# jialeli1/From-Voxel-to-Point

Measured on AMD Instinct MI355X. Metric: point clouds/sec fwd+bwd (FV2P, KITTI shape) at 1/2/4/8 MI355X, higher is better.
Workload: dtype f32

## Files before the change

from-voxel-to-point_amd/csrc/roi_pool.hip:

```cpp
#include "common.hpp"
#include "../../include/fv2p_math.h"

namespace fv2p {

FV2P_HD int pt_in_box3d(const float* pt, const float* box, float margin, float* local_x, float* local_y) {
  const float x = pt[0], y = pt[1], z = pt[2];
  const float cx = box[0], cy = box[1], cz = box[2];
  const float dx = box[3], dy = box[4], dz = box[5], rz = box[6];
  if (static_cast<double>(fabsf(z - cz)) > static_cast<double>(dz) / 2.0) return 0;
  const float sx = x - cx, sy = y - cy;
  const float cosa = fv2p_cosf(-rz), sina = fv2p_sinf(-rz);
  const float lx = sx * cosa + sy * (-sina);
  const float ly = sx * sina + sy * cosa;
  *local_x = lx;
  *local_y = ly;
  const bool in_x = static_cast<double>(fabsf(lx)) < static_cast<double>(dx) / 2.0 + static_cast<double>(margin);
  const bool in_y = static_cast<double>(fabsf(ly)) < static_cast<double>(dy) / 2.0 + static_cast<double>(margin);
  return in_x && in_y;
}

constexpr float kMarginGpu = 1e-5f;
constexpr float kMarginCpu = 1e-2f;

__global__ __launch_bounds__(256) void points_in_boxes_k(int boxes_num, int pts_num, const float* __restrict__ boxes,
// ... 9 lines not shown
  int idx = -1;
  float lx, ly;
  for (int k = 0; k < boxes_num; ++k)
    if (pt_in_box3d(pt, sbox + k * 7, kMarginGpu, &lx, &ly)) { idx = k; break; }
  out[static_cast<int64_t>(b) * pts_num + i] = idx;
}

constexpr int kRoiPoolWaves = 16;
__device__ __forceinline__ int roi_pool_select(int pts_num, int sampled, int row, const float* __restrict__ xyz_b, const float* box, int* sidx,
                                               int* wave_cnt, float* __restrict__ dst, int* __restrict__ empty_flag) {
  constexpr int T = kRoiPoolWaves * 64;
  const int lane = threadIdx.x & 63, w = threadIdx.x >> 6;
  int total = 0;
  for (int base = 0; base < pts_num && total < sampled; base += T) {
    const int i = base + threadIdx.x;
    int in = 0;
    if (i < pts_num) {
      const float* p = xyz_b + static_cast<int64_t>(i) * 3;
      const float pt[3] = {p[0], p[1], p[2]};
      float lx, ly;
      in = pt_in_box3d(pt, box, kMarginGpu, &lx, &ly);
    }
    const uint64_t vote = __ballot(in);
    if (lane == 0) wave_cnt[w] = __popcll(vote);
    __syncthreads();
    int pos = total + __popcll(vote & lanemask_lt()), all = 0;
#pragma unroll
    for (int ww = 0; ww < kRoiPoolWaves; ++ww) { const int c = wave_cnt[ww]; if (ww < w) pos += c; all += c; }
    if (in && pos < sampled) sidx[pos] = i;
    total += all;
    __syncthreads();
  }
  const int cnt = total < sampled ? total : sampled;
  if (threadIdx.x == 0) *empty_flag = (cnt == 0) ? 1 : 0;
  if (cnt == 0)
    for (int e = threadIdx.x; e < sampled * row; e += T) dst[e] = 0.f;
  return cnt;
}

__global__ __launch_bounds__(kRoiPoolWaves * 64) void roipoint_pool_k(int pts_num, int boxes_num, int feat_len, int sampled, const float* __restrict__ xyz,
                                                       const float* __restrict__ boxes3d, const float* __restrict__ feats,
                                                       float* __restrict__ pooled, int* __restrict__ empty_flag) {
  extern __shared__ int sidx[];
  __shared__ int wave_cnt[kRoiPoolWaves];
  const int m = blockIdx.x, b = blockIdx.y;
  const int lane = threadIdx.x & 63, w = threadIdx.x >> 6;
  float box[7];
  for (int j = 0; j < 7; ++j) box[j] = boxes3d[(static_cast<int64_t>(b) * boxes_num + m) * 7 + j];
  const int row = 3 + feat_len;
  float* dst = pooled + (static_cast<int64_t>(b) * boxes_num + m) * sampled * row;
  const int cnt = roi_pool_select(pts_num, sampled, row, xyz + static_cast<int64_t>(b) * pts_num * 3, box, sidx, wave_cnt, dst,
                                  empty_flag + static_cast<int64_t>(b) * boxes_num + m);
  if (cnt == 0) return;
  const float* fx = xyz + static_cast<int64_t>(b) * pts_num * 3;
  const float* ff = feats + static_cast<int64_t>(b) * pts_num * feat_len;
  for (int s0 = 4 * w; s0 < sampled; s0 += 4 * kRoiPoolWaves) {
    int src[4];
#pragma unroll
    for (int u = 0; u < 4; ++u) { const int sl = s0 + u < sampled ? s0 + u : sampled - 1; src[u] = sidx[sl < cnt ? sl : sl % cnt]; }
    for (int j0 = 0; j0 < row; j0 += 128) {
      float v[4][2];
#pragma unroll
      for (int u = 0; u < 4; ++u)
#pragma unroll
        for (int q = 0; q < 2; ++q) {
          const int j = j0 + 64 * q + lane;
          v[u][q] = j < 3 ? fx[static_cast<int64_t>(src[u]) * 3 + j] : (j < row ? ff[static_cast<int64_t>(src[u]) * feat_len + (j - 3)] : 0.f);
// ... 30 lines not shown
  const float ca = cosf(-roi[6]), sa = sinf(-roi[6]);
  const float* fs = score + static_cast<int64_t>(b) * pts_num;
  const float* ff = feats + static_cast<int64_t>(b) * pts_num * feat_len;
  for (int s0 = 4 * w; s0 < sampled; s0 += 4 * kRoiPoolWaves) {
    int src[4];
    float head[4];
#pragma unroll
    for (int u = 0; u < 4; ++u) { const int sl = s0 + u < sampled ? s0 + u : sampled - 1; src[u] = sidx[sl < cnt ? sl : sl % cnt]; }
#pragma unroll
    for (int u = 0; u < 4; ++u) {
      const float* p = fx + static_cast<int64_t>(src[u]) * 3;
      const float x = p[0], y = p[1], z = p[2], sc = fs[src[u]];
      const float dx = x - roi[0], dy = y - roi[1];
      head[u] = lane == 0 ? dx * ca - dy * sa : (lane == 1 ? dx * sa + dy * ca : (lane == 2 ? z - roi[2] : (lane == 3 ? sc : sqrtf(x * x + y * y + z * z) / depth_norm - 0.5f)));
    }
    for (int j0 = 0; j0 < row; j0 += 128) {
      float v[4][2];
#pragma unroll
      for (int u = 0; u < 4; ++u)
#pragma unroll
        for (int q = 0; q < 2; ++q) {
          const int j = j0 + 64 * q + lane;
          const float f = (j >= 5 && j < row) ? ff[static_cast<int64_t>(src[u]) * feat_len + (j - 5)] : 0.f;
          v[u][q] = j < 5 ? head[u] : f;
        }
#pragma unroll
      for (int u = 0; u < 4; ++u)
#pragma unroll
        for (int q = 0; q < 2; ++q) {
          const int j = j0 + 64 * q + lane;
          if (j < row && s0 + u < sampled) dst[static_cast<int64_t>(s0 + u) * row + j] = v[u][q];
        }
    }
  }
}

__global__ __launch_bounds__(64) void roiaware_collect_k(int pts_num, int max_pts, int out_x, int out_y, int out_z,
                                                         const float* __restrict__ rois, const float* __restrict__ pts,
                                                         int* __restrict__ pts_idx_of_voxels) {
  extern __shared__ int s_cnt[];
  const int box_idx = blockIdx.x, lane = threadIdx.x;
  const int nvox = out_x * out_y * out_z;
  for (int e = lane; e < nvox; e += 64) s_cnt[e] = 0;
  __builtin_amdgcn_wave_barrier();
  float box[7];
  for (int j = 0; j < 7; ++j) box[j] = rois[box_idx * 7 + j];
  int* vox = pts_idx_of_voxels + static_cast<int64_t>(box_idx) * nvox * max_pts;
  const int max_num = max_pts - 1;
  const float dx = box[3], dy = box[4], dz = box[5];
  const float x_res = dx / out_x, y_res = dy / out_y, z_res = dz / out_z;
  for (int base = 0; base < pts_num; base += 64) {
    const int i = base + lane;
    int in = 0, v = -1;
    if (i < pts_num) {
      const float pt[3] = {pts[i * 3], pts[i * 3 + 1], pts[i * 3 + 2]};
      float lx = 0.f, ly = 0.f;
      in = pt_in_box3d(pt, box, kMarginGpu, &lx, &ly);
      if (in) {
        const float lz = pt[2] - box[2];
        int xi = static_cast<int>((lx + dx / 2) / x_res);
        int yi = static_cast<int>((ly + dy / 2) / y_res);
        int zi = static_cast<int>((lz + dz / 2) / z_res);
        xi = min(max(xi, 0), out_x - 1);
        yi = min(max(yi, 0), out_y - 1);
        zi = min(max(zi, 0), out_z - 1);
        v = (xi * out_y + yi) * out_z + zi;
// ... 119 lines not shown
                                    fv2p_stream_t stream_) {
  hipStream_t stream = static_cast<hipStream_t>(stream_);
  FV2P_REQUIRE(batch >= 0 && pts_num >= 0 && boxes_num >= 0 && feature_len >= 0 && sampled_pts_num >= 1, FV2P_EINVAL,
               "roipoint_pool3d: bad sizes");
  if (batch == 0 || boxes_num == 0) return 0;
  FV2P_REQUIRE(boxes3d && pooled_features && pooled_empty_flag && (xyz || pts_num == 0) && (pts_feature || feature_len == 0 || pts_num == 0),
               FV2P_EINVAL, "roipoint_pool3d: null pointer");
  FV2P_REQUIRE(static_cast<size_t>(sampled_pts_num) * 4 <= 60000, FV2P_ELIMIT, "roipoint_pool3d: sampled_pts_num > 15000");
  hipLaunchKernelGGL(roipoint_pool_k, dim3(boxes_num, batch), dim3(kRoiPoolWaves * 64), sampled_pts_num * sizeof(int), stream, pts_num, boxes_num,
                     feature_len, sampled_pts_num, xyz, boxes3d, pts_feature, pooled_features, pooled_empty_flag);
  FV2P_LAUNCH_CHECK();
  return 0;
}

extern "C" int fv2p_roipoint_pool3d_frame(const float* xyz, const float* pts_score, const float* pts_feature, const float* boxes3d,
                                          const float* rois, int batch, int pts_num, int boxes_num, int feature_len, int sampled_pts_num,
                                          float depth_normalizer, float* pooled_features, int* pooled_empty_flag, fv2p_stream_t stream_) {
  hipStream_t stream = static_cast<hipStream_t>(stream_);
  FV2P_REQUIRE(batch >= 0 && pts_num >= 0 && boxes_num >= 0 && feature_len >= 0 && sampled_pts_num >= 1, FV2P_EINVAL,
               "roipoint_pool3d_frame: bad sizes");
  FV2P_REQUIRE(depth_normalizer > 0.f, FV2P_EINVAL, "roipoint_pool3d_frame: depth_normalizer must be positive");
  if (batch == 0 || boxes_num == 0) return 0;
  FV2P_REQUIRE(boxes3d && rois && pooled_features && pooled_empty_flag && ((xyz && pts_score) || pts_num == 0) &&
               (pts_feature || feature_len == 0 || pts_num == 0), FV2P_EINVAL, "roipoint_pool3d_frame: null pointer");
  FV2P_REQUIRE(static_cast<size_t>(sampled_pts_num) * 4 <= 60000, FV2P_ELIMIT, "roipoint_pool3d_frame: sampled_pts_num > 15000");
  FV2P_REQUIRE(static_cast<int64_t>(sampled_pts_num) * (5 + feature_len) < (1ll << 31), FV2P_ELIMIT, "roipoint_pool3d_frame: a RoI's rows exceed 2^31 values");
  hipLaunchKernelGGL(roipoint_pool_frame_k, dim3(boxes_num, batch), dim3(kRoiPoolWaves * 64), sampled_pts_num * sizeof(int), stream, pts_num,
                     boxes_num, feature_len, sampled_pts_num, depth_normalizer, xyz, pts_score, pts_feature, boxes3d, rois, pooled_features,
                     pooled_empty_flag);
  FV2P_LAUNCH_CHECK();
  return 0;
}

extern "C" int fv2p_roiaware_pool3d_fwd(const float* rois, const float* pts, const float* pts_feature, int boxes_num, int pts_num,
                                        int channels, int max_pts_each_voxel, int out_x, int out_y, int out_z, int pool_method,
                                        int* argmax, int* pts_idx_of_voxels, float* pooled_features, fv2p_stream_t stream_) {
  hipStream_t stream = static_cast<hipStream_t>(stream_);
  FV2P_REQUIRE(boxes_num >= 0 && pts_num >= 0 && channels >= 1 && max_pts_each_voxel >= 2, FV2P_EINVAL, "roiaware_pool3d: bad sizes");
  FV2P_REQUIRE(out_x >= 1 && out_y >= 1 && out_z >= 1 && out_x < 256 && out_y < 256 && out_z < 256, FV2P_EINVAL,
               "roiaware_pool3d: out size must be in [1,255] (roiaware_pool3d.cpp:53)");
  FV2P_REQUIRE(pool_method == 0 || pool_method == 1, FV2P_EINVAL, "roiaware_pool3d: pool_method must be 0 (max) or 1 (avg)");
  FV2P_REQUIRE(static_cast<int64_t>(out_x) * out_y * out_z * 4 <= 64000, FV2P_ELIMIT, "roiaware_pool3d: more than 16000 voxels per RoI");
  if (boxes_num == 0) return 0;
  FV2P_REQUIRE(rois && argmax && pts_idx_of_voxels && pooled_features && (pts || pts_num == 0), FV2P_EINVAL, "roiaware_pool3d: null pointer");
  const int64_t voxels = static_cast<int64_t>(boxes_num) * out_x * out_y * out_z;
  FV2P_HIP(hipMemsetAsync(pts_idx_of_voxels, 0, sizeof(int) * voxels * max_pts_each_voxel, stream));
  FV2P_HIP(hipMemsetAsync(pooled_features, 0, sizeof(float) * voxels * channels, stream));
  FV2P_HIP(hipMemsetAsync(argmax, 0, sizeof(int) * voxels * channels, stream));
  if (pts_num > 0)
    hipLaunchKernelGGL(roiaware_collect_k, dim3(boxes_num), dim3(64), sizeof(int) * out_x * out_y * out_z, stream, pts_num, max_pts_each_voxel, out_x, out_y, out_z, rois, pts,
                       pts_idx_of_voxels);
  const int64_t total = voxels * channels;
  const dim3 grid(static_cast<unsigned>(ceil_div(total, 256))), block(256);
  if (pool_method == 0)
    hipLaunchKernelGGL(roiaware_pool_k<0>, grid, block, 0, stream, total, channels, max_pts_each_voxel, pts_feature, pts_idx_of_voxels,
                       pooled_features, argmax);
  else
    hipLaunchKernelGGL(roiaware_pool_k<1>, grid, block, 0, stream, total, channels, max_pts_each_voxel, pts_feature, pts_idx_of_voxels,
                       pooled_features, argmax);
  FV2P_LAUNCH_CHECK();
  return 0;
}

extern "C" int fv2p_roiaware_pool3d_bwd(const int* pts_idx_of_voxels, const int* argmax, const float* grad_out, int boxes_num, int out_x,
                                        int out_y, int out_z, int channels, int max_pts_each_voxel, int pool_method, float* grad_in,
                                        fv2p_stream_t stream_) {
// ... 50 lines not shown
```

from-voxel-to-point_amd/fv2p_harness/fv2p_model.py:

```python
import math
import os
from functools import partial

import numpy as np
import torch
import torch.nn as nn
import torch.nn.functional as F

from pcdet.ops.iou3d_nms import iou3d_nms_cuda, iou3d_nms_utils
from pcdet.ops.pointnet2.pointnet2_batch import pointnet2_modules as pn2_batch_modules
from pcdet.ops.pointnet2.pointnet2_batch import fused as pn2_fused
from pcdet.ops.pointnet2.pointnet2_batch import pointnet2_utils as pn2_batch
from pcdet.ops.pointnet2.pointnet2_stack import pointnet2_utils as pn2_stack
from pcdet.ops.roiaware_pool3d import roiaware_pool3d_utils
from pcdet.ops.roipoint_pool3d import roipoint_pool3d_utils
from pcdet.models.backbones_3d.pfe import bev_grid_pooling
from pcdet.ops.spconv import norm as _norm
from pcdet.ops.spconv import head as _head
from pcdet.ops.spconv import linear as _linear
from pcdet.ops.spconv import bev_entry as _bev_entry

import fv2p_native as _nat

from .backbone import VoxelResBackBone8x, bn_act
# ... 265 lines not shown


class PointLossFn(torch.autograd.Function):

    @staticmethod
    def forward(ctx, logits, labels, weight):
        logits, labels = logits.contiguous(), labels.contiguous()
        n = logits.numel()
        out = logits.new_empty(1)
        dlogits, score = torch.empty_like(logits), logits.new_empty(n)
        with _nat.device_guard(logits.device):
            ws = _nat.workspace(int(_nat.lib().fv2p_point_loss_ws_bytes(n)), logits.device)
            _nat.call("fv2p_point_loss", logits, labels, n, 0.25, float(weight), out, dlogits, score, ws, ws.numel(), _nat.stream())
        ctx.save_for_backward(dlogits)
        ctx.mark_non_differentiable(score)
        return out[0], score

    @staticmethod
    def backward(ctx, g, _):
        dlogits, = ctx.saved_tensors
        return dlogits * g, None, None


def roi_grid_geometry(rois, g):
    if not (rois.is_cuda and rois.dtype == torch.float32) or rois.requires_grad:
        raise ValueError("roi_grid_geometry: float32 CUDA rois without gradient (IoUGuidedRoIHead.grid_points is the tensor form)")
    r = rois.reshape(-1, 7).contiguous()
    local, column, corners = r.new_empty(r.shape[0], g ** 3, 3), r.new_empty(r.shape[0], g * g, 3), r.new_empty(r.shape[0], 8, 3)
    with _nat.device_guard(r.device):
        _nat.call("fv2p_roi_grid", r, r.shape[0], g, local, column, corners, _nat.stream())
    return local, column, corners


def pool_points_in_frame(layer, depth_normalizer, key, feats, scores, rois):
    with torch.no_grad():
        b, n, _ = key.shape
        m, c, s = rois.shape[1], feats.shape[1], layer.num_sampled_points
        rois = rois.contiguous()
        big, extra = rois.clone(), layer.pool_extra_width
        if isinstance(extra, (list, tuple)) and len(set(extra)) == 1:
            big[..., 3:6] += extra[0]
        elif isinstance(extra, (list, tuple)):
            for axis, e in enumerate(extra):
                big[..., 3 + axis] += e
        else:
            big[..., 3:6] += rois[..., 3:6] * extra
        pooled = feats.new_empty((b * m, s, 5 + c))
        empty = torch.empty((b, m), dtype=torch.int32, device=feats.device)
        with _nat.device_guard(feats.device):
            _nat.call("fv2p_roipoint_pool3d_frame", key.contiguous(), scores.detach().contiguous(), feats.detach().contiguous(), big, rois,
                      b, n, m, c, s, float(depth_normalizer), pooled, empty, _nat.stream())
    return pooled


class AnchorHead(nn.Module):

    def __init__(self, cfg, cin):
        super().__init__()
        self.cfg = cfg
        nr, nc = len(cfg.anchor_rotations), len(cfg.anchor_classes)
        na = nr * nc
        self.conv_cls = nn.Conv2d(cin, na, 1)
        self.conv_box = nn.Conv2d(cin, na * 7, 1)
        self.conv_dir_cls = nn.Conv2d(cin, na * cfg.num_dir_bins, 1)
        nn.init.constant_(self.conv_cls.bias, -math.log((1 - 0.01) / 0.01))
        nn.init.normal_(self.conv_box.weight, mean=0, std=0.001)
        r = cfg.point_cloud_range
        w, h = cfg.grid_size[0] // 8, cfg.grid_size[1] // 8
        xs = torch.arange(r[0], r[3] + 1e-5, step=(r[3] - r[0]) / (w - 1), dtype=torch.float32)
        ys = torch.arange(r[1], r[4] + 1e-5, step=(r[4] - r[1]) / (h - 1), dtype=torch.float32)
        a = torch.zeros(h, w, nc, nr, 7)
        a[..., 0] = xs.view(1, w, 1, 1)
        a[..., 1] = ys.view(h, 1, 1, 1)
        for c, (size, bottom, _, _) in enumerate(cfg.anchor_classes):
            a[:, :, c, :, 3:6] = torch.tensor(size)
            a[:, :, c, :, 2] = bottom
        a[..., 6] = torch.tensor(cfg.anchor_rotations).view(1, 1, 1, nr)
        a[..., 2] += a[..., 5] / 2
        self.register_buffer("anchors", a.view(-1, 7), persistent=False)
        self.register_buffer("anchor_rot", a.view(-1, 7)[:, 6].contiguous(), persistent=False)
        for c in range(nc):
            ac = a[:, :, c].reshape(-1, 7).contiguous()
            self.register_buffer(f"anchors_c{c}", ac, persistent=False)
            self.register_buffer(f"anchor_bev_c{c}", nearest_bev_boxes(ac), persistent=False)

# ... 452 lines not shown
    def roi_streams(self, bev, s_rois, bev_stride=8):
        b = bev.shape[0]
        g = self.cfg.grid_size_roi
        kernel = KERNEL_GLUE and s_rois.is_cuda and s_rois.dtype == torch.float32 and not s_rois.requires_grad
        if kernel:
            local, column, corners = roi_grid_geometry(s_rois, g)
        else:
            world, local = self.grid_points(s_rois)
            column = world.view(world.shape[0], g * g, g, 3)[:, :, 0] if KERNEL_GLUE and world.shape[1] == g ** 3 else None
        n_roi = local.shape[0]
        batch_dict = {"batch_size": b, "spatial_features_before_head": bev, "spatial_features_stride": bev_stride}
        if column is not None:
            g_bev = self.bev_grid_pool_layer(batch_dict, column.reshape(b, -1, 3))
            g_bev = g_bev.view(n_roi, g * g, 1, -1).expand(-1, -1, g, -1).reshape(n_roi, g ** 3, -1)
        else:
            g_bev = self.bev_grid_pool_layer(batch_dict, world.view(b, -1, 3)).view(world.shape[0], world.shape[1], -1)
        g_bev = g_bev.permute(0, 2, 1).contiguous()
        if not kernel:
            t = dconst(s_rois, _CORNER_SIGNS, s_rois.dtype) / 2
            corners = s_rois.reshape(-1, 7)[:, None, 3:6] * t[None]
        cge = self.cge_inter(self.cge_up(corners.transpose(1, 2).unsqueeze(3).contiguous()).squeeze(-1))
        return dict(local=local, g_bev=g_bev, cge=cge)

    def finish(self, key, feats, scores, prep):
        rois = prep["s_rois"]
        cls, reg = self.predict(key, feats, scores, rois, prep)
        if KERNEL_GLUE and cls.is_cuda:
            loss = self.losses(rois, prep["s_gt"], prep["gt_ct"], prep["s_iou"], cls, reg, None)
        else:
            loss = self.losses(rois, prep["s_gt"], prep["gt_ct"], prep["s_iou"], cls, reg[:, 1:], reg[:, :1])
        return loss, {"rois": prep["rois"], "sampled_rois": rois, "roi_iou": prep["s_iou"]}

    def predict(self, key, feats, scores, rois, prep):
        pooled = self.pool_points(key, feats, scores, rois)
        h = pooled[..., 0:5]
        for layer in self.xyz_up_layer:
            h = rows_linear(h, layer.weight, layer.bias) if isinstance(layer, nn.Conv2d) else layer(h)
        h = torch.cat((h, pooled[..., 5:]), dim=2)
        for layer in self.merge_down_layer:
            h = rows_linear(h, layer.weight, layer.bias) if isinstance(layer, nn.Conv2d) else layer(h)
        g_pt = sa_msg_grid(self.SA_modules[0], pooled[..., 0:3].contiguous(), None, prep["local"].contiguous(), rows=h)
        grid = torch.cat((g_pt, prep["g_bev"]), dim=1)
        pc = self.grid_interact_fc_layer(grid.view(grid.shape[0], -1, 1))
        shared = self.feature_fusion(torch.cat((pc, prep["cge"]), dim=1))
        cls = self.cls_layers(shared).squeeze(-1)
        reg = self.reg_layers(shared).squeeze(-1)
        return cls, reg

    @staticmethod
    def reg_losses(rois, gt_src, gt_ct, fg, reg):
        n_fg = fg.sum().clamp_min(1.0)
        r7 = rois.reshape(-1, 7)
        anchor = torch.cat((torch.zeros_like(r7[:, :3]), r7[:, 3:6], torch.zeros_like(r7[:, 6:7])), dim=1)
        target = residual_encode(gt_ct.reshape(-1, gt_ct.shape[-1])[:, :7], anchor)
        loss_reg = (smooth_l1(reg - target, 1.0 / 9.0) * fg[:, None]).sum() / n_fg
        local = residual_decode(reg, anchor)
        world = rotate_z(local.unsqueeze(1), r7[:, 6]).squeeze(1)
        world = torch.cat((world[:, :3] + r7[:, :3], world[:, 3:6], world[:, 6:7] + r7[:, 6:7]), dim=1)
        g = gt_src.reshape(-1, gt_src.shape[-1])[:, :7]
        loss_corner = (corner_loss_lidar(world, g) * fg).sum() / n_fg
        return loss_reg, loss_corner

    def losses(self, rois, gt_src, gt_ct, iou, cls, reg, iou_pred):
        cfg = self.cfg
        if KERNEL_GLUE and cls.is_cuda and cls.dtype == torch.float32:
            return RoiLossFn.apply(rois, gt_src, iou, cls, reg if iou_pred is None else torch.cat((iou_pred, reg), dim=1), cfg)
        if iou_pred is None:
            reg, iou_pred = reg[:, 1:], reg[:, :1]
        if gt_ct is None:
            gt_ct = self.canonical_targets(rois.reshape(1, -1, 7), gt_src.reshape(1, -1, gt_src.shape[-1]))
        iou = iou.view(-1)
        soft = ((iou - cfg.cls_bg) / (cfg.cls_fg - cfg.cls_bg)).clamp(0, 1)
        soft = torch.where(iou > cfg.cls_fg, torch.ones_like(soft), torch.where(iou < cfg.cls_bg, torch.zeros_like(soft), soft))
        loss_cls = F.binary_cross_entropy(torch.sigmoid(cls.view(-1)), soft, reduction="none").mean()
        fg = (iou > cfg.reg_fg).float()
        loss_reg, loss_corner = self.reg_losses(rois, gt_src, gt_ct, fg, reg)
        lab = (iou - 0.5) * 2
        valid = (lab >= (cfg.reg_fg - 0.5) * 2).float()
        loss_iou = (F.smooth_l1_loss(iou_pred.view(-1), lab, reduction="none") * valid).sum() / valid.sum().clamp_min(1.0)
        return loss_cls + loss_reg + loss_corner + loss_iou
# ... 95 lines not shown
```

include/fv2p_ops.h:

```cpp
#ifndef FV2P_OPS_H_
#define FV2P_OPS_H_

#include <stddef.h>
#include <stdint.h>

#ifdef __cplusplus
extern "C" {
#endif

#define FV2P_ABI_VERSION 1

#define FV2P_EINVAL      (-1)
#define FV2P_EWORKSPACE  (-2)
#define FV2P_EHIP        (-3)
#define FV2P_ELIMIT      (-4)

typedef void* fv2p_stream_t;

const char* fv2p_last_error(void);
int fv2p_abi_version(void);

size_t fv2p_scan_ws_bytes(int64_t n);
int fv2p_exclusive_scan_i32(const int* in, int* out, int64_t n, int* total, void* ws, size_t ws_bytes,
                            fv2p_stream_t stream);
// ... 197 lines not shown
int fv2p_roi_sample_targets(const float* iou, const float* rois, const float* gt, const float* uniforms, int batch, int r, int g, int n,
                            int gt_w, float fg_thresh, float bg_lo, float reg_fg, int fg_quota, float hard_ratio, float* s_rois,
                            float* s_gt, float* s_iou, int* s_index, fv2p_stream_t stream);

size_t fv2p_anchor_assign_ws_bytes(int batch, int g);
int fv2p_anchor_assign(const float* anchor_bev, const float* anchors, int n_anchor, const float* gt_bev, const float* gt, int batch, int g,
                       int gt_w, float matched_thr, float unmatched_thr, int* labels, float* reg, void* ws, size_t ws_bytes,
                       fv2p_stream_t stream);

size_t fv2p_anchor_loss_ws_bytes(int batch, int n_anchor);
int fv2p_anchor_loss(const float* cls, const float* box, const float* dirs, const int* labels, const float* reg_t, const float* anchor_rot,
                     int batch, int n_anchor, float alpha, float beta, float dir_offset, float w_cls, float w_loc, float w_dir, float* loss4,
                     float* dcls, float* dbox, float* ddirs, void* ws, size_t ws_bytes, fv2p_stream_t stream);

int fv2p_roi_loss(const float* rois, const float* gt, const float* iou, const float* cls, const float* reg, int r, int gt_w, float cls_fg,
                  float cls_bg, float soft_span, float reg_fg, float iou_label_thr, float beta, float* loss5, float* dcls, float* dreg,
                  float* canonical, fv2p_stream_t stream);

size_t fv2p_point_loss_ws_bytes(int n);
int fv2p_point_loss(const float* logits, const int64_t* labels, int n, float alpha, float weight, float* loss, float* dlogits, float* score,
                    void* ws, size_t ws_bytes, fv2p_stream_t stream);

int fv2p_roi_grid(const float* rois, int r, int g, float* local, float* column, float* corners, fv2p_stream_t stream);

int fv2p_points_in_boxes(const float* boxes, const float* pts, int batch, int boxes_num, int pts_num,
                         int* box_idx_of_points, fv2p_stream_t stream);
int fv2p_points_in_boxes_cpu(const float* boxes, const float* pts, int boxes_num, int pts_num, int* pts_indices);
int fv2p_roipoint_pool3d(const float* xyz, const float* boxes3d, const float* pts_feature, int batch, int pts_num,
                         int boxes_num, int feature_len, int sampled_pts_num, float* pooled_features,
                         int* pooled_empty_flag, fv2p_stream_t stream);
int fv2p_roipoint_pool3d_frame(const float* xyz, const float* pts_score, const float* pts_feature, const float* boxes3d,
                               const float* rois, int batch, int pts_num, int boxes_num, int feature_len, int sampled_pts_num,
                               float depth_normalizer, float* pooled_features, int* pooled_empty_flag, fv2p_stream_t stream);
int fv2p_roiaware_pool3d_fwd(const float* rois, const float* pts, const float* pts_feature, int boxes_num,
                             int pts_num, int channels, int max_pts_each_voxel, int out_x, int out_y, int out_z,
                             int pool_method, int* argmax, int* pts_idx_of_voxels, float* pooled_features,
                             fv2p_stream_t stream);
int fv2p_roiaware_pool3d_bwd(const int* pts_idx_of_voxels, const int* argmax, const float* grad_out, int boxes_num,
                             int out_x, int out_y, int out_z, int channels, int max_pts_each_voxel, int pool_method,
                             float* grad_in, fv2p_stream_t stream);
size_t fv2p_roiaware_pool3d_bwd_ws_bytes(int boxes_num, int out_x, int out_y, int out_z, int channels, int max_pts_each_voxel,
                                         int pool_method);
int fv2p_roiaware_pool3d_bwd_gather(const int* pts_idx_of_voxels, const int* argmax, const float* grad_out, int boxes_num,
                                    int out_x, int out_y, int out_z, int channels, int max_pts_each_voxel, int pool_method,
                                    int pts_num, float* grad_in, void* ws, size_t ws_bytes, fv2p_stream_t stream);

int fv2p_ball_query_batch(int b, int n, int m, float radius, int nsample, const float* new_xyz, const float* xyz,
                          int* idx, fv2p_stream_t stream);
int fv2p_ball_query_stack(int b, int m, float radius, int nsample, const float* new_xyz,
                          const int* new_xyz_batch_cnt, const float* xyz, const int* xyz_batch_cnt, int* idx,
                          fv2p_stream_t stream);
int fv2p_voxel_query_stack(int m, int r1, int r2, int r3, int nsample, float radius, int z_range, int y_range,
                           int x_range, const float* new_xyz, const float* xyz, const int* new_coords,
                           const int* point_indices, int* idx, fv2p_stream_t stream);
int fv2p_group_points_batch(int b, int c, int n, int npoints, int nsample, const float* points, const int* idx,
                            float* out, fv2p_stream_t stream);
int fv2p_group_points_batch_grad(int b, int c, int n, int npoints, int nsample, const float* grad_out,
                                 const int* idx, float* grad_points, fv2p_stream_t stream);
int fv2p_gather_points(int b, int c, int n, int npoints, const float* points, const int* idx, float* out,
                       fv2p_stream_t stream);
int fv2p_gather_points_grad(int b, int c, int n, int npoints, const float* grad_out, const int* idx,
                            float* grad_points, fv2p_stream_t stream);
int fv2p_group_points_stack(int b, int m, int c, int nsample, const float* features,
                            const int* features_batch_cnt, const int* idx, const int* idx_batch_cnt, float* out,
                            fv2p_stream_t stream);
int fv2p_group_points_stack_grad(int b, int m, int c, int n, int nsample, const float* grad_out, const int* idx,
// ... 279 lines not shown
int fv2p_linear_bn_backward_h(const void* x, const void* z, const void* dy, int64_t n, int cin, const void* w, int cout,
                              const float* mean, const float* invstd, const void* gamma, const void* beta, int relu,
                              int batch_stats, void* du, void* dx, void* dw, void* dgamma, void* dbeta, int dt, int wd, int pd,
                              void* ws, size_t ws_bytes, fv2p_stream_t stream);

int fv2p_voxel_pool_supported(int64_t m, int s, int c);
int fv2p_voxel_pool_blocks(int64_t m);
size_t fv2p_voxel_pool_saved_bytes(int c);
size_t fv2p_voxel_pool_ws_bytes(int64_t m, int s, int c);
size_t fv2p_voxel_pool_backward_ws_bytes(int64_t m, int s, int c, int64_t n);
int fv2p_voxel_pool_forward(const float* f, const float* xyz, const float* new_xyz, const int* idx, const unsigned char* empty,
                            int64_t n, int64_t m, int s, int c, const float* w, const float* gamma, const float* beta,
                            float* running_mean, float* running_var, int64_t* num_batches_tracked, float momentum, float eps,
                            int training, float* out, unsigned char* arg, double* saved, void* ws, size_t ws_bytes,
                            fv2p_stream_t stream);
int fv2p_voxel_pool_backward(const float* xyz, const float* new_xyz, const int* idx, const unsigned char* empty, int64_t n,
                             int64_t m, int s, int c, const float* w, const float* gamma, const float* out,
                             const unsigned char* arg, const double* saved, const float* grad_out, int training, float* grad_f,
                             float* grad_w, float* grad_gamma, float* grad_beta, void* ws, size_t ws_bytes,
                             fv2p_stream_t stream);

size_t fv2p_voxel_pool_backward_h_ws_bytes(int64_t m, int s, int c, int64_t n);
int fv2p_voxel_pool_forward_h(const void* f, const float* xyz, const float* new_xyz, const int* idx, const unsigned char* empty,
                              int64_t n, int64_t m, int s, int c, const float* w, const float* gamma, const float* beta,
                              float* running_mean, float* running_var, int64_t* num_batches_tracked, float momentum, float eps,
                              int training, void* out, unsigned char* arg, double* saved, void* ws, size_t ws_bytes, int dtype,
                              fv2p_stream_t stream);
int fv2p_voxel_pool_backward_h(const float* xyz, const float* new_xyz, const int* idx, const unsigned char* empty, int64_t n,
                               int64_t m, int s, int c, const float* w, const float* gamma, const void* out,
                               const unsigned char* arg, const double* saved, const void* grad_out, int training, void* grad_f,
                               float* grad_w, float* grad_gamma, float* grad_beta, void* ws, size_t ws_bytes, int dtype,
                               fv2p_stream_t stream);

#ifdef __cplusplus
}
#endif
#endif
```

Before: 121.5.

## Pool RoI point indices and split merge-down linear to skip feature gather

Adds an index-only RoI point pooling kernel that writes the 5 geometric channels plus a source index instead of copying the full per-point feature rows. The merge_down linear over the concatenated features is split algebraically: the feature half is applied once per source point and gathered by index inside a fused bias+add+ReLU kernel. Also adds fused affine+ReLU and bias+ReLU row kernels with double-accumulated weight/bias gradients, and a scatter-add backward for the gathered term. This avoids materialising and multiplying a large duplicated pooled-feature tensor, at the cost of a longer set of eligibility checks and a scatter-add in backward.

```diff
diff --git a/from-voxel-to-point_amd/csrc/roi_pool.hip b/from-voxel-to-point_amd/csrc/roi_pool.hip
--- a/from-voxel-to-point_amd/csrc/roi_pool.hip
+++ b/from-voxel-to-point_amd/csrc/roi_pool.hip
@@ -65,7 +65,7 @@
     __syncthreads();
   }
   const int cnt = total < sampled ? total : sampled;
-  if (threadIdx.x == 0) *empty_flag = (cnt == 0) ? 1 : 0;
+  if (threadIdx.x == 0 && empty_flag) *empty_flag = (cnt == 0) ? 1 : 0;
   if (cnt == 0)
     for (int e = threadIdx.x; e < sampled * row; e += T) dst[e] = 0.f;
   return cnt;
@@ -162,6 +162,45 @@
           if (j < row && s0 + u < sampled) dst[static_cast<int64_t>(s0 + u) * row + j] = v[u][q];
         }
     }
+  }
+}
+
+__global__ __launch_bounds__(kRoiPoolWaves * 64) void roipoint_pool_frame_idx_k(int pts_num, int boxes_num, int sampled, float depth_norm,
+                                                       const float* __restrict__ xyz, const float* __restrict__ score,
+                                                       const float* __restrict__ boxes_big, const float* __restrict__ rois,
+                                                       float* __restrict__ geo, int* __restrict__ idx, int* __restrict__ empty_flag) {
+  extern __shared__ int sidx[];
+  __shared__ int wave_cnt[kRoiPoolWaves];
+  constexpr int T = kRoiPoolWaves * 64;
+  const int m = blockIdx.x, b = blockIdx.y;
+  const int64_t r = static_cast<int64_t>(b) * boxes_num + m;
+  float box[7], roi[7];
+  for (int j = 0; j < 7; ++j) {
+    box[j] = boxes_big[r * 7 + j];
+    roi[j] = rois[r * 7 + j];
+  }
+  float* dst = geo + r * sampled * 5;
+  int* di = idx + r * sampled;
+  const float* fx = xyz + static_cast<int64_t>(b) * pts_num * 3;
+  const int cnt = roi_pool_select(pts_num, sampled, 5, fx, box, sidx, wave_cnt, dst, empty_flag ? empty_flag + r : nullptr);
+  if (cnt == 0) {
+    for (int k = threadIdx.x; k < sampled; k += T) di[k] = -1;
+    return;
+  }
+  const float ca = cosf(-roi[6]), sa = sinf(-roi[6]);
+  const float* fs = score + static_cast<int64_t>(b) * pts_num;
+  for (int k = threadIdx.x; k < sampled; k += T) {
+    const int src = sidx[k < cnt ? k : k % cnt];
+    const float* p = fx + static_cast<int64_t>(src) * 3;
+    const float x = p[0], y = p[1], z = p[2], sc = fs[src];
+    const float dx = x - roi[0], dy = y - roi[1];
+    float* o = dst + static_cast<int64_t>(k) * 5;
+    o[0] = dx * ca - dy * sa;
+    o[1] = dx * sa + dy * ca;
+    o[2] = z - roi[2];
+    o[3] = sc;
+    o[4] = sqrtf(x * x + y * y + z * z) / depth_norm - 0.5f;
+    di[k] = b * pts_num + src;
   }
 }
 
@@ -347,6 +386,22 @@
   return 0;
 }
 
+extern "C" int fv2p_roipoint_pool3d_frame_idx(const float* xyz, const float* pts_score, const float* boxes3d, const float* rois, int batch,
+                                              int pts_num, int boxes_num, int sampled_pts_num, float depth_normalizer, float* geo, int* idx,
+                                              int* pooled_empty_flag, fv2p_stream_t stream_) {
+  hipStream_t stream = static_cast<hipStream_t>(stream_);
+  FV2P_REQUIRE(batch >= 0 && pts_num >= 0 && boxes_num >= 0 && sampled_pts_num >= 1, FV2P_EINVAL, "roipoint_pool3d_frame_idx: bad sizes");
+  FV2P_REQUIRE(depth_normalizer > 0.f, FV2P_EINVAL, "roipoint_pool3d_frame_idx: depth_normalizer must be positive");
+  if (batch == 0 || boxes_num == 0) return 0;
+  FV2P_REQUIRE(boxes3d && rois && geo && idx && ((xyz && pts_score) || pts_num == 0), FV2P_EINVAL, "roipoint_pool3d_frame_idx: null pointer");
+  FV2P_REQUIRE(static_cast<size_t>(sampled_pts_num) * 4 <= 60000, FV2P_ELIMIT, "roipoint_pool3d_frame_idx: sampled_pts_num > 15000");
+  FV2P_REQUIRE(static_cast<int64_t>(batch) * pts_num < (1ll << 31), FV2P_ELIMIT, "roipoint_pool3d_frame_idx: 2^31 points or more");
+  hipLaunchKernelGGL(roipoint_pool_frame_idx_k, dim3(boxes_num, batch), dim3(kRoiPoolWaves * 64), sampled_pts_num * sizeof(int), stream, pts_num,
+                     boxes_num, sampled_pts_num, depth_normalizer, xyz, pts_score, boxes3d, rois, geo, idx, pooled_empty_flag);
+  FV2P_LAUNCH_CHECK();
+  return 0;
+}
+
 extern "C" int fv2p_roiaware_pool3d_fwd(const float* rois, const float* pts, const float* pts_feature, int boxes_num, int pts_num,
                                         int channels, int max_pts_each_voxel, int out_x, int out_y, int out_z, int pool_method,
                                         int* argmax, int* pts_idx_of_voxels, float* pooled_features, fv2p_stream_t stream_) {
diff --git a/from-voxel-to-point_amd/csrc/roi_rows.hip b/from-voxel-to-point_amd/csrc/roi_rows.hip
--- /dev/null
+++ b/from-voxel-to-point_amd/csrc/roi_rows.hip
@@ -0,0 +1,299 @@
+#include "common.hpp"
+
+namespace fv2p {
+
+constexpr int kRowsThreads = 256;
+constexpr int kRowsMaxC = 1024;
+constexpr int kRowsMaxK = 8;
+constexpr int kRowsFwdIter = 4;
+constexpr int kRowsBwdBlocks = 2048;
+
+static inline bool rows_shape_ok(int64_t n, int c, int k) {
+  return n >= 1 && n < (1ll << 31) && c >= 4 && c <= kRowsMaxC && c % 4 == 0 && k >= 0 && k <= kRowsMaxK;
+}
+static inline int64_t rows_bwd_span(int64_t n, int c) {
+  const int rpp = kRowsThreads / (c / 4);
+  int64_t iter = ceil_div(n, static_cast<int64_t>(rpp) * kRowsBwdBlocks);
+  iter = ceil_div(iter < 4 ? 4 : iter, 4) * 4;
+  return iter * rpp;
+}
+static inline bool aligned16(const void* p) { return (reinterpret_cast<uintptr_t>(p) & 15) == 0; }
+
+__device__ __forceinline__ float relu1(float v) { return v < 0.f ? 0.f : v; }
+
+__global__ __launch_bounds__(kRowsThreads) void rows_bias_relu_fwd_k(int64_t n, int c, const float* z, const float* __restrict__ bias,
+                                                                     const float* __restrict__ g, const int* __restrict__ idx, int64_t g_rows,
+                                                                     float* y) {
+  const int cq = c >> 2, rpp = kRowsThreads / cq;
+  const int cg = threadIdx.x % cq, rl = threadIdx.x / cq;
+  if (rl >= rpp) return;
+  const float4 b4 = *reinterpret_cast<const float4*>(bias + 4 * cg);
+  const int64_t r0 = static_cast<int64_t>(blockIdx.x) * rpp * kRowsFwdIter + rl;
+  float4 v[kRowsFwdIter], a[kRowsFwdIter];
+#pragma unroll
+  for (int u = 0; u < kRowsFwdIter; ++u) {
+    const int64_t r = r0 + static_cast<int64_t>(u) * rpp;
+    v[u] = make_float4(0.f, 0.f, 0.f, 0.f);
+    a[u] = v[u];
+    if (r < n) {
+      v[u] = *reinterpret_cast<const float4*>(z + r * c + 4 * cg);
+      const int64_t i = g ? static_cast<int64_t>(idx[r]) : -1;
+      if (i >= 0 && i < g_rows) a[u] = *reinterpret_cast<const float4*>(g + i * c + 4 * cg);
+    }
+  }
+#pragma unroll
+  for (int u = 0; u < kRowsFwdIter; ++u) {
+    const int64_t r = r0 + static_cast<int64_t>(u) * rpp;
+    if (r < n) {
+      float4 o;
+      o.x = relu1((v[u].x + b4.x) + a[u].x);
+      o.y = relu1((v[u].y + b4.y) + a[u].y);
+      o.z = relu1((v[u].z + b4.z) + a[u].z);
+      o.w = relu1((v[u].w + b4.w) + a[u].w);
+      *reinterpret_cast<float4*>(y + r * c + 4 * cg) = o;
+    }
+  }
+}
+
+__device__ __forceinline__ void rows_block_sum(const double (&acc)[4], bool active, int c, int rpp, int rl, int cg, double* red,
+                                               double* __restrict__ part) {
+  if (active) {
+#pragma unroll
+    for (int u = 0; u < 4; ++u) red[rl * c + 4 * cg + u] = acc[u];
+  }
+  __syncthreads();
+  for (int col = threadIdx.x; col < c; col += kRowsThreads) {
+    double s = 0.0;
+    for (int q = 0; q < rpp; ++q) s += red[q * c + col];
+    part[col] = s;
+  }
+  __syncthreads();
+}
+
+__global__ __launch_bounds__(kRowsThreads) void rows_bias_relu_bwd_k(int64_t n, int c, int64_t span, const float* dy, const float* __restrict__ y,
+                                                                     float* dz, double* __restrict__ part) {
+  __shared__ double red[kRowsMaxC];
+  const int cq = c >> 2, rpp = kRowsThreads / cq;
+  const int cg = threadIdx.x % cq, rl = threadIdx.x / cq;
+  const bool active = rl < rpp;
+  const int64_t begin = static_cast<int64_t>(blockIdx.x) * span;
+  const int64_t end = begin + span < n ? begin + span : n;
+  double acc[4] = {0.0, 0.0, 0.0, 0.0};
+  if (active)
+    for (int64_t rb = begin + rl; rb < end; rb += 4ll * rpp) {
+      float4 d[4], o[4];
+#pragma unroll
+      for (int u = 0; u < 4; ++u) {
+        const int64_t r = rb + static_cast<int64_t>(u) * rpp;
+        d[u] = make_float4(0.f, 0.f, 0.f, 0.f);
+        o[u] = d[u];
+        if (r < end) {
+          d[u] = *reinterpret_cast<const float4*>(dy + r * c + 4 * cg);
+          o[u] = *reinterpret_cast<const float4*>(y + r * c + 4 * cg);
+        }
+      }
+#pragma unroll
+      for (int u = 0; u < 4; ++u) {
+        const int64_t r = rb + static_cast<int64_t>(u) * rpp;
+        if (r < end) {
+          float4 q;
+          q.x = o[u].x > 0.f ? d[u].x : 0.f;
+          q.y = o[u].y > 0.f ? d[u].y : 0.f;
+          q.z = o[u].z > 0.f ? d[u].z : 0.f;
+          q.w = o[u].w > 0.f ? d[u].w : 0.f;
+          *reinterpret_cast<float4*>(dz + r * c + 4 * cg) = q;
+          acc[0] += static_cast<double>(q.x);
+          acc[1] += static_cast<double>(q.y);
+          acc[2] += static_cast<double>(q.z);
+          acc[3] += static_cast<double>(q.w);
+        }
+      }
+    }
+  rows_block_sum(acc, active, c, rpp, rl, cg, red, part + static_cast<int64_t>(blockIdx.x) * c);
+}
+
+__global__ __launch_bounds__(64) void rows_fold_k(int64_t blocks, int c, int groups, const double* __restrict__ part, float* __restrict__ dw,
+                                                  float* __restrict__ db) {
+  const int j = blockIdx.x, lane = threadIdx.x;
+  const int64_t stride = static_cast<int64_t>(c) * groups;
+  double s = 0.0;
+  for (int64_t b0 = lane; b0 < blocks; b0 += 64 * 8) {
+    double v[8];
+#pragma unroll
+    for (int u = 0; u < 8; ++u) { const int64_t b = b0 + 64 * u; v[u] = b < blocks ? part[b * stride + j] : 0.0; }
+#pragma unroll
+    for (int u = 0; u < 8; ++u) s += v[u];
+  }
+#pragma unroll
+  for (int off = 32; off >= 1; off >>= 1) s += __shfl_down(s, off, 64);
+  if (lane == 0) {
+    const int q = j / c, col = j % c;
+    if (q == groups - 1) { if (db) db[col] = static_cast<float>(s); }
+    else if (dw) dw[static_cast<int64_t>(col) * (groups - 1) + q] = static_cast<float>(s);
+  }
+}
+
+template <int K>
+__global__ __launch_bounds__(kRowsThreads) void rows_affine_relu_fwd_k(int64_t n, int c, const float* __restrict__ x, const float* __restrict__ w,
+                                                                       const float* __restrict__ bias, float* __restrict__ y) {
+  const int cq = c >> 2, rpp = kRowsThreads / cq;
+  const int cg = threadIdx.x % cq, rl = threadIdx.x / cq;
+  if (rl >= rpp) return;
+  float wr[4][K];
+#pragma unroll
+  for (int u = 0; u < 4; ++u)
+#pragma unroll
+    for (int i = 0; i < K; ++i) wr[u][i] = w[static_cast<int64_t>(4 * cg + u) * K + i];
+  const float4 b4 = *reinterpret_cast<const float4*>(bias + 4 * cg);
+  const int64_t r0 = static_cast<int64_t>(blockIdx.x) * rpp * kRowsFwdIter + rl;
+#pragma unroll
+  for (int u = 0; u < kRowsFwdIter; ++u) {
+    const int64_t r = r0 + static_cast<int64_t>(u) * rpp;
+    if (r < n) {
+      float xr[K];
+#pragma unroll
+      for (int i = 0; i < K; ++i) xr[i] = x[r * K + i];
+      float o[4];
+#pragma unroll
+      for (int v = 0; v < 4; ++v) {
+        float a = xr[0] * wr[v][0];
+#pragma unroll
+        for (int i = 1; i < K; ++i) a = fmaf(xr[i], wr[v][i], a);
+        o[v] = a;
+      }
+      *reinterpret_cast<float4*>(y + r * c + 4 * cg) = make_float4(relu1(o[0] + b4.x), relu1(o[1] + b4.y), relu1(o[2] + b4.z), relu1(o[3] + b4.w));
+    }
+  }
+}
+
+template <int K>
+__global__ __launch_bounds__(kRowsThreads) void rows_affine_relu_bwd_k(int64_t n, int c, int64_t span, const float* __restrict__ dy,
+                                                                       const float* __restrict__ y, const float* __restrict__ x,
+                                                                       double* __restrict__ part) {
+  __shared__ double red[kRowsMaxC];
+  const int cq = c >> 2, rpp = kRowsThreads / cq;
+  const int cg = threadIdx.x % cq, rl = threadIdx.x / cq;
+  const bool active = rl < rpp;
+  const int64_t begin = static_cast<int64_t>(blockIdx.x) * span;
+  const int64_t end = begin + span < n ? begin + span : n;
+  double acc[K + 1][4];
+#pragma unroll
+  for (int i = 0; i <= K; ++i)
+#pragma unroll
+    for (int u = 0; u < 4; ++u) acc[i][u] = 0.0;
+  if (active)
+    for (int64_t rb = begin + rl; rb < end; rb += 2ll * rpp) {
+      float4 d[2], o[2];
+      float xr[2][K];
+#pragma unroll
+      for (int u = 0; u < 2; ++u) {
+        const int64_t r = rb + static_cast<int64_t>(u) * rpp;
+        d[u] = make_float4(0.f, 0.f, 0.f, 0.f);
+        o[u] = d[u];
+#pragma unroll
+        for (int i = 0; i < K; ++i) xr[u][i] = 0.f;
+        if (r < end) {
+          d[u] = *reinterpret_cast<const float4*>(dy + r * c + 4 * cg);
+          o[u] = *reinterpret_cast<const float4*>(y + r * c + 4 * cg);
+#pragma unroll
+          for (int i = 0; i < K; ++i) xr[u][i] = x[r * K + i];
+        }
+      }
+#pragma unroll
+      for (int u = 0; u < 2; ++u) {
+        const int64_t r = rb + static_cast<int64_t>(u) * rpp;
+        if (r < end) {
+          const double q[4] = {o[u].x > 0.f ? static_cast<double>(d[u].x) : 0.0, o[u].y > 0.f ? static_cast<double>(d[u].y) : 0.0,
+                               o[u].z > 0.f ? static_cast<double>(d[u].z) : 0.0, o[u].w > 0.f ? static_cast<double>(d[u].w) : 0.0};
+#pragma unroll
+          for (int i = 0; i < K; ++i) {
+            const double xv = static_cast<double>(xr[u][i]);
+#pragma unroll
+            for (int v = 0; v < 4; ++v) acc[i][v] += q[v] * xv;
+          }
+#pragma unroll
+          for (int v = 0; v < 4; ++v) acc[K][v] += q[v];
+        }
+      }
+    }
+  double* out = part + static_cast<int64_t>(blockIdx.x) * (K + 1) * c;
+#pragma unroll
+  for (int i = 0; i <= K; ++i) rows_block_sum(acc[i], active, c, rpp, rl, cg, red, out + static_cast<int64_t>(i) * c);
+}
+
+}
+using namespace fv2p;
+
+#define FV2P_ROWS_K(k, CALL)                                                                                                         \
+  switch (k) { case 1: CALL(1) break; case 2: CALL(2) break; case 3: CALL(3) break; case 4: CALL(4) break; case 5: CALL(5) break;    \
+               case 6: CALL(6) break; case 7: CALL(7) break; default: CALL(8) }
+
+extern "C" int fv2p_rows_supported(int64_t n, int c, int k) { return rows_shape_ok(n, c, k) ? 1 : 0; }
+
+extern "C" size_t fv2p_rows_bwd_ws_bytes(int64_t n, int c, int k) {
+  if (!rows_shape_ok(n, c, k)) return 0;
+  return align_up(static_cast<size_t>(ceil_div(n, rows_bwd_span(n, c))) * c * (k + 1) * sizeof(double));
+}
+
+extern "C" int fv2p_rows_affine_relu_forward(const float* x, const float* w, const float* bias, int64_t n, int k, int c, float* y,
+                                             fv2p_stream_t stream_) {
+  FV2P_REQUIRE(rows_shape_ok(n, c, k) && k >= 1, FV2P_ELIMIT, "rows_affine_relu_forward: shape (n %lld, k %d, c %d) is not taken",
+               static_cast<long long>(n), k, c);
+  FV2P_REQUIRE(x && w && bias && y, FV2P_EINVAL, "rows_affine_relu_forward: null pointer");
+  FV2P_REQUIRE(aligned16(bias) && aligned16(y), FV2P_EINVAL, "rows_affine_relu_forward: bias and y must be 16-byte aligned");
+  hipStream_t stream = static_cast<hipStream_t>(stream_);
+  const int rpp = kRowsThreads / (c / 4);
+  const dim3 grid(static_cast<unsigned>(ceil_div(n, static_cast<int64_t>(rpp) * kRowsFwdIter)));
+#define FV2P_CALL(K) hipLaunchKernelGGL(rows_affine_relu_fwd_k<K>, grid, dim3(kRowsThreads), 0, stream, n, c, x, w, bias, y);
+  FV2P_ROWS_K(k, FV2P_CALL)
+#undef FV2P_CALL
+  FV2P_LAUNCH_CHECK();
+  return 0;
+}
+
+extern "C" int fv2p_rows_affine_relu_backward(const float* dy, const float* y, const float* x, int64_t n, int k, int c, float* dw, float* db,
+                                              void* ws, size_t ws_bytes, fv2p_stream_t stream_) {
+  FV2P_REQUIRE(rows_shape_ok(n, c, k) && k >= 1, FV2P_ELIMIT, "rows_affine_relu_backward: shape (n %lld, k %d, c %d) is not taken",
+               static_cast<long long>(n), k, c);
+  FV2P_REQUIRE(dy && y && x && dw && db, FV2P_EINVAL, "rows_affine_relu_backward: null pointer");
+  FV2P_REQUIRE(aligned16(dy) && aligned16(y), FV2P_EINVAL, "rows_affine_relu_backward: dy and y must be 16-byte aligned");
+  FV2P_REQUIRE(ws && ws_bytes >= fv2p_rows_bwd_ws_bytes(n, c, k), FV2P_EWORKSPACE, "rows_affine_relu_backward: workspace too small");
+  hipStream_t stream = static_cast<hipStream_t>(stream_);
+  const int64_t span = rows_bwd_span(n, c), blocks = ceil_div(n, span);
+  double* part = static_cast<double*>(ws);
+#define FV2P_CALL(K) hipLaunchKernelGGL(rows_affine_relu_bwd_k<K>, dim3(static_cast<unsigned>(blocks)), dim3(kRowsThreads), 0, stream, n, c, span, dy, y, x, part);
+  FV2P_ROWS_K(k, FV2P_CALL)
+#undef FV2P_CALL
+  hipLaunchKernelGGL(rows_fold_k, dim3(static_cast<unsigned>(c * (k + 1))), dim3(64), 0, stream, blocks, c, k + 1, part, dw, db);
+  FV2P_LAUNCH_CHECK();
+  return 0;
+}
+
+extern "C" int fv2p_rows_bias_relu_forward(const float* z, const float* bias, const float* g, const int* idx, int64_t g_rows, int64_t n, int c,
+                                           float* y, fv2p_stream_t stream_) {
+  FV2P_REQUIRE(rows_shape_ok(n, c, 0), FV2P_ELIMIT, "rows_bias_relu_forward: shape (n %lld, c %d) is not taken", static_cast<long long>(n), c);
+  FV2P_REQUIRE(z && bias && y && (!g || (idx && g_rows >= 0)), FV2P_EINVAL, "rows_bias_relu_forward: null pointer");
+  FV2P_REQUIRE(aligned16(z) && aligned16(bias) && aligned16(y) && aligned16(g), FV2P_EINVAL,
+               "rows_bias_relu_forward: z, bias, g and y must be 16-byte aligned");
+  hipStream_t stream = static_cast<hipStream_t>(stream_);
+  const int rpp = kRowsThreads / (c / 4);
+  hipLaunchKernelGGL(rows_bias_relu_fwd_k, dim3(static_cast<unsigned>(ceil_div(n, static_cast<int64_t>(rpp) * kRowsFwdIter))), dim3(kRowsThreads), 0,
+                     stream, n, c, z, bias, g, idx, g_rows, y);
+  FV2P_LAUNCH_CHECK();
+  return 0;
+}
+
+extern "C" int fv2p_rows_bias_relu_backward(const float* dy, const float* y, int64_t n, int c, float* dz, float* db, void* ws, size_t ws_bytes,
+                                            fv2p_stream_t stream_) {
+  FV2P_REQUIRE(rows_shape_ok(n, c, 0), FV2P_ELIMIT, "rows_bias_relu_backward: shape (n %lld, c %d) is not taken", static_cast<long long>(n), c);
+  FV2P_REQUIRE(dy && y && dz && db, FV2P_EINVAL, "rows_bias_relu_backward: null pointer");
+  FV2P_REQUIRE(aligned16(dy) && aligned16(y) && aligned16(dz), FV2P_EINVAL, "rows_bias_relu_backward: dy, y and dz must be 16-byte aligned");
+  FV2P_REQUIRE(ws && ws_bytes >= fv2p_rows_bwd_ws_bytes(n, c, 0), FV2P_EWORKSPACE, "rows_bias_relu_backward: workspace too small");
+  hipStream_t stream = static_cast<hipStream_t>(stream_);
+  const int64_t span = rows_bwd_span(n, c), blocks = ceil_div(n, span);
+  double* part = static_cast<double*>(ws);
+  hipLaunchKernelGGL(rows_bias_relu_bwd_k, dim3(static_cast<unsigned>(blocks)), dim3(kRowsThreads), 0, stream, n, c, span, dy, y, dz, part);
+  hipLaunchKernelGGL(rows_fold_k, dim3(static_cast<unsigned>(c)), dim3(64), 0, stream, blocks, c, 1, part, nullptr, db);
+  FV2P_LAUNCH_CHECK();
+  return 0;
+}
diff --git a/from-voxel-to-point_amd/fv2p_harness/fv2p_model.py b/from-voxel-to-point_amd/fv2p_harness/fv2p_model.py
--- a/from-voxel-to-point_amd/fv2p_harness/fv2p_model.py
+++ b/from-voxel-to-point_amd/fv2p_harness/fv2p_model.py
@@ -321,25 +321,109 @@
     return local, column, corners
 
 
+def enlarged_boxes(layer, rois):
+    big, extra = rois.clone(), layer.pool_extra_width
+    if isinstance(extra, (list, tuple)) and len(set(extra)) == 1:
+        big[..., 3:6] += extra[0]
+    elif isinstance(extra, (list, tuple)):
+        for axis, e in enumerate(extra):
+            big[..., 3 + axis] += e
+    else:
+        big[..., 3:6] += rois[..., 3:6] * extra
+    return big
+
+
 def pool_points_in_frame(layer, depth_normalizer, key, feats, scores, rois):
     with torch.no_grad():
         b, n, _ = key.shape
         m, c, s = rois.shape[1], feats.shape[1], layer.num_sampled_points
         rois = rois.contiguous()
-        big, extra = rois.clone(), layer.pool_extra_width
-        if isinstance(extra, (list, tuple)) and len(set(extra)) == 1:
-            big[..., 3:6] += extra[0]
-        elif isinstance(extra, (list, tuple)):
-            for axis, e in enumerate(extra):
-                big[..., 3 + axis] += e
-        else:
-            big[..., 3:6] += rois[..., 3:6] * extra
+        big = enlarged_boxes(layer, rois)
         pooled = feats.new_empty((b * m, s, 5 + c))
         empty = torch.empty((b, m), dtype=torch.int32, device=feats.device)
         with _nat.device_guard(feats.device):
             _nat.call("fv2p_roipoint_pool3d_frame", key.contiguous(), scores.detach().contiguous(), feats.detach().contiguous(), big, rois,
                       b, n, m, c, s, float(depth_normalizer), pooled, empty, _nat.stream())
     return pooled
+
+
+def pool_point_rows_in_frame(layer, depth_normalizer, key, scores, rois):
+    with torch.no_grad():
+        b, n, _ = key.shape
+        m, s = rois.shape[1], layer.num_sampled_points
+        rois = rois.contiguous()
+        big = enlarged_boxes(layer, rois)
+        geo = key.new_empty((b * m, s, 5))
+        idx = torch.empty((b * m, s), dtype=torch.int32, device=key.device)
+        with _nat.device_guard(key.device):
+            _nat.call("fv2p_roipoint_pool3d_frame_idx", key.contiguous(), scores.detach().contiguous(), big, rois, b, n, m, s,
+                      float(depth_normalizer), geo, idx, None, _nat.stream())
+    return geo, idx
+
+
+def rows_kernels_take(n, c, k=0):
+    return bool(_nat.lib().fv2p_rows_supported(n, c, k))
+
+
+class RowsAffineReluFn(torch.autograd.Function):
+
+    @staticmethod
+    def forward(ctx, x, weight, bias):
+        x, w, bias = x.contiguous(), weight.reshape(weight.shape[0], -1).contiguous(), bias.contiguous()
+        n, k, c = x.shape[0], x.shape[1], w.shape[0]
+        y = x.new_empty((n, c))
+        with _nat.device_guard(x.device):
+            _nat.call("fv2p_rows_affine_relu_forward", x, w, bias, n, k, c, y, _nat.stream())
+        ctx.save_for_backward(x, y)
+        ctx.w_shape = weight.shape
+        return y
+
+    @staticmethod
+    def backward(ctx, dy):
+        x, y = ctx.saved_tensors
+        n, k, c = x.shape[0], x.shape[1], y.shape[1]
+        dy = dy.contiguous()
+        dw, db = y.new_empty((c, k)), y.new_empty(c)
+        with _nat.device_guard(y.device):
+            ws = _nat.workspace(int(_nat.lib().fv2p_rows_bwd_ws_bytes(n, c, k)), y.device)
+            _nat.call("fv2p_rows_affine_relu_backward", dy, y, x, n, k, c, dw, db, ws, ws.numel(), _nat.stream())
+        return None, dw.view(ctx.w_shape), db
+
+
+class RowsBiasReluFn(torch.autograd.Function):
+
+    @staticmethod
+    def forward(ctx, z, bias, g, idx):
+        c = z.shape[-1]
+        n = z.numel() // c
+        if not z.is_contiguous():
+            raise ValueError("RowsBiasReluFn: z must be contiguous (it is overwritten)")
+        bias = bias.contiguous()
+        if g is not None:
+            g, idx = g.contiguous(), idx.contiguous()
+        with _nat.device_guard(z.device):
+            _nat.call("fv2p_rows_bias_relu_forward", z, bias, g, idx, 0 if g is None else g.shape[0], n, c, z, _nat.stream())
+        ctx.mark_dirty(z)
+        ctx.save_for_backward(z, idx)
+        ctx.g_rows = None if g is None else g.shape[0]
+        return z
+
+    @staticmethod
+    def backward(ctx, dy):
+        y, idx = ctx.saved_tensors
+        c = y.shape[-1]
+        n = y.numel() // c
+        dy = dy.contiguous()
+        dz, db = torch.empty_like(dy), y.new_empty(c)
+        dg = None
+        with _nat.device_guard(y.device):
+            ws = _nat.workspace(int(_nat.lib().fv2p_rows_bwd_ws_bytes(n, c, 0)), y.device)
+            _nat.call("fv2p_rows_bias_relu_backward", dy, y, n, c, dz, db, ws, ws.numel(), _nat.stream())
+            if ctx.g_rows is not None and ctx.needs_input_grad[2]:
+                dg = y.new_zeros((ctx.g_rows, c))
+                ws = _nat.workspace(int(_nat.lib().fv2p_scatter_add_ws_bytes(n, c)), y.device)
+                _nat.call("fv2p_scatter_add", n, c, ctx.g_rows, idx, None, None, dz, 1, dg, ws, ws.numel(), _nat.stream())
+        return dz, db, dg, None
 
 
 class AnchorHead(nn.Module):
@@ -858,20 +942,55 @@
         return loss, {"rois": prep["rois"], "sampled_rois": rois, "roi_iou": prep["s_iou"]}
 
     def predict(self, key, feats, scores, rois, prep):
-        pooled = self.pool_points(key, feats, scores, rois)
-        h = pooled[..., 0:5]
-        for layer in self.xyz_up_layer:
-            h = rows_linear(h, layer.weight, layer.bias) if isinstance(layer, nn.Conv2d) else layer(h)
-        h = torch.cat((h, pooled[..., 5:]), dim=2)
-        for layer in self.merge_down_layer:
-            h = rows_linear(h, layer.weight, layer.bias) if isinstance(layer, nn.Conv2d) else layer(h)
-        g_pt = sa_msg_grid(self.SA_modules[0], pooled[..., 0:3].contiguous(), None, prep["local"].contiguous(), rows=h)
+        if self.point_rows_route(key, feats, scores, rois):
+            geo, h = self.point_rows(key, feats, scores, rois)
+            xyz = geo[..., 0:3].contiguous()
+        else:
+            pooled = self.pool_points(key, feats, scores, rois)
+            h = pooled[..., 0:5]
+            for layer in self.xyz_up_layer:
+                h = rows_linear(h, layer.weight, layer.bias) if isinstance(layer, nn.Conv2d) else layer(h)
+            h = torch.cat((h, pooled[..., 5:]), dim=2)
+            for layer in self.merge_down_layer:
+                h = rows_linear(h, layer.weight, layer.bias) if isinstance(layer, nn.Conv2d) else layer(h)
+            xyz = pooled[..., 0:3].contiguous()
+        g_pt = sa_msg_grid(self.SA_modules[0], xyz, None, prep["local"].contiguous(), rows=h)
         grid = torch.cat((g_pt, prep["g_bev"]), dim=1)
         pc = self.grid_interact_fc_layer(grid.view(grid.shape[0], -1, 1))
         shared = self.feature_fusion(torch.cat((pc, prep["cge"]), dim=1))
         cls = self.cls_layers(shared).squeeze(-1)
         reg = self.reg_layers(shared).squeeze(-1)
         return cls, reg
+
+    def point_rows_route(self, key, feats, scores, rois):
+        up, down = self.xyz_up_layer, self.merge_down_layer
+        if not (KERNEL_GLUE and key.is_cuda and feats.is_cuda and scores.is_cuda and key.dtype == feats.dtype == torch.float32
+                and not torch.is_autocast_enabled() and len(up) == 4 and len(down) == 2):
+            return False
+        convs, relus = (up[0], up[2], down[0]), (up[1], up[3], down[1])
+        plain = all(not (m._forward_hooks or m._forward_pre_hooks or m._backward_hooks or m._backward_pre_hooks or "forward" in m.__dict__)
+                    for m in (up, down) + convs + relus)
+        if not (plain and all(type(m) is nn.Conv2d and m.kernel_size == (1, 1) and m.groups == 1 and m.bias is not None
+                              and m.weight.is_cuda and m.weight.dtype == torch.float32 for m in convs)
+                and all(type(m) is nn.ReLU for m in relus)):
+            return False
+        c = up[0].out_channels
+        return (up[0].in_channels == 5 and (up[2].in_channels, up[2].out_channels) == (c, c) and feats.dim() == 2 and feats.shape[1] == c
+                and (down[0].in_channels, down[0].out_channels) == (2 * c, c)
+                and rows_kernels_take(max(rois.numel() // 7, 1) * self.roipoint_pool3d_layer.num_sampled_points, c, 5))
+
+    def point_rows(self, key, feats, scores, rois):
+        geo, idx = pool_point_rows_in_frame(self.roipoint_pool3d_layer, self.cfg.depth_normalizer, key, scores, rois)
+        up, down = self.xyz_up_layer, self.merge_down_layer
+        r, s, c = geo.shape[0], geo.shape[1], up[0].out_channels
+        h = RowsAffineReluFn.apply(geo.view(r * s, 5), up[0].weight, up[0].bias).view(r, s, c)
+        h = RowsBiasReluFn.apply(rows_linear(h, up[2].weight), up[2].bias, None, None)
+        w3 = down[0].weight.reshape(c, 2 * c)
+        rows = feats.shape[0]
+        chunk = s if s > 0 and rows % s == 0 else max(rows, 1)
+        per_key = rows_linear(feats.detach().reshape(-1, chunk, c), w3[:, c:]).view(rows, c)
+        h = RowsBiasReluFn.apply(rows_linear(h, w3[:, :c]), down[0].bias, per_key, idx.view(-1))
+        return geo, h
 
     @staticmethod
     def reg_losses(rois, gt_src, gt_ct, fg, reg):
diff --git a/include/fv2p_ops.h b/include/fv2p_ops.h
--- a/include/fv2p_ops.h
+++ b/include/fv2p_ops.h
@@ -253,6 +253,9 @@
 int fv2p_roipoint_pool3d_frame(const float* xyz, const float* pts_score, const float* pts_feature, const float* boxes3d,
                                const float* rois, int batch, int pts_num, int boxes_num, int feature_len, int sampled_pts_num,
                                float depth_normalizer, float* pooled_features, int* pooled_empty_flag, fv2p_stream_t stream);
+int fv2p_roipoint_pool3d_frame_idx(const float* xyz, const float* pts_score, const float* boxes3d, const float* rois, int batch,
+                                   int pts_num, int boxes_num, int sampled_pts_num, float depth_normalizer, float* geo, int* idx,
+                                   int* pooled_empty_flag, fv2p_stream_t stream);
 int fv2p_roiaware_pool3d_fwd(const float* rois, const float* pts, const float* pts_feature, int boxes_num,
                              int pts_num, int channels, int max_pts_each_voxel, int out_x, int out_y, int out_z,
                              int pool_method, int* argmax, int* pts_idx_of_voxels, float* pooled_features,
@@ -598,6 +601,17 @@
                                float* grad_w, float* grad_gamma, float* grad_beta, void* ws, size_t ws_bytes, int dtype,
                                fv2p_stream_t stream);
 
+int fv2p_rows_supported(int64_t n, int c, int k);
+size_t fv2p_rows_bwd_ws_bytes(int64_t n, int c, int k);
+int fv2p_rows_affine_relu_forward(const float* x, const float* w, const float* bias, int64_t n, int k, int c, float* y,
+                                  fv2p_stream_t stream);
+int fv2p_rows_affine_relu_backward(const float* dy, const float* y, const float* x, int64_t n, int k, int c, float* dw, float* db,
+                                   void* ws, size_t ws_bytes, fv2p_stream_t stream);
+int fv2p_rows_bias_relu_forward(const float* z, const float* bias, const float* g, const int* idx, int64_t g_rows, int64_t n, int c,
+                                float* y, fv2p_stream_t stream);
+int fv2p_rows_bias_relu_backward(const float* dy, const float* y, int64_t n, int c, float* dz, float* db, void* ws, size_t ws_bytes,
+                                 fv2p_stream_t stream);
+
 #ifdef __cplusplus
 }
 #endif
```

New measurement: 110.7. 8.9% lower.
